# ethz-asl/ethzasl_brisk

Measured on AMD Instinct MI355X. Metric: frames/sec detect+describe @1080p (1/2/4/8 GPU); % HBM roofline, higher is better.
Workload: dtype u8

## Files before the change

ethzasl_brisk_amd/csrc/brisk_device_detect.h:

```cpp
#pragma once
#include "brisk_common.h"

BRISK_HD int brisk_min(int a, int b) { return a < b ? a : b; }
BRISK_HD int brisk_max(int a, int b) { return a > b ? a : b; }
BRISK_HD int brisk_min3(int a, int b, int c) { return brisk_min(brisk_min(a, b), c); }
BRISK_HD int brisk_max3(int a, int b, int c) { return brisk_max(brisk_max(a, b), c); }

struct BriskScoreBlock {
  uint32_t w0, w1, w2, w3;
  int x0, y0, cw, ch;
};

struct BriskLayerView {
  const uint8_t* img;
  uint16_t* smap;
  int w, h, stride;
  BriskScoreBlock blk;
  BriskScoreBlock blk58;
  mutable int miss;
};

BRISK_HD void brisk_block_clear(BriskScoreBlock* b) { b->w0 = b->w1 = b->w2 = b->w3 = 0; b->x0 = b->y0 = b->cw = b->ch = 0; }
BRISK_HD void brisk_block_from_bytes(BriskScoreBlock* b, const uint8_t* v, int n, int x0, int y0, int cw, int ch) {
  uint32_t w[4] = {0, 0, 0, 0};
  for (int i = 0; i < n; ++i) w[i >> 2] |= (uint32_t)v[i] << (8 * (i & 3));
  b->w0 = w[0]; b->w1 = w[1]; b->w2 = w[2]; b->w3 = w[3];
  b->x0 = x0; b->y0 = y0; b->cw = cw; b->ch = ch;
}
BRISK_HD int brisk_block_get(const BriskScoreBlock& b, int idx) {
  const uint32_t w = (idx < 8) ? ((idx < 4) ? b.w0 : b.w1) : ((idx < 12) ? b.w2 : b.w3);
  return (int)((w >> ((idx & 3) * 8)) & 0xFFu);
}

#if defined(__HIPCC__)
#ifdef BRISK_OUTLINE_HELPERS
#define BRISK_HD_OUTLINE __host__ __device__ static __attribute__((noinline))
#else
#define BRISK_HD_OUTLINE __host__ __device__ static inline
#endif
#else
#define BRISK_HD_OUTLINE static
#endif


BRISK_HD int brisk_avg(int a, int b) { return (a + b + 1) >> 1; }

BRISK_HD uint8_t brisk_half_px(const uint8_t* src, int sstride, int sw, int c, int r) {
  const uint8_t* p1 = src + (long)(2 * r) * sstride + 2 * c;
  const uint8_t* p2 = p1 + sstride;
  const int hsize = sw / 16;
  const int n1 = 16 * (hsize / 2);
  const int n2 = n1 + 8 * (hsize % 2);
  const int a = p1[0], b = p1[1], cc = p2[0], d = p2[1];
  if (c < n2) {
    const int v0 = brisk_avg(a, cc), v1 = brisk_avg(b, d);
    return (uint8_t)(c < n1 ? brisk_avg(v0, v1) : (v0 + v1) / 2);
  }
  return (uint8_t)((a + b + cc + d + 2) / 4);
}

BRISK_HD uint8_t brisk_twothird_px(const uint8_t* src, int sstride, int sw, int c, int r) {
  const int t = c >> 1, cx = c & 1;
  const int g = r >> 1, ry = r & 1;
  const uint8_t* pa = src + (long)(3 * g + (ry ? 2 : 0)) * sstride + 3 * t;
  const uint8_t* pb = src + (long)(3 * g + 1) * sstride + 3 * t;
  const int simd_cols = (sw / 15) * 10;
  const int o = cx ? 2 : 0;
  if (c < simd_cols) {
    const int uo = brisk_avg(brisk_avg(pa[o], pb[o]), pa[o]);
    const int um = brisk_avg(brisk_avg(pa[1], pb[1]), pa[1]);
    return (uint8_t)brisk_avg(brisk_avg(uo, um), uo);
  }
  const unsigned A1 = pa[o], A2 = pa[1], B1 = pb[o], B2 = pb[1];
  return (uint8_t)(((4 * A1 + 2 * (A2 + B1 + 1) + B2 + 1) / 9) & 0xFF);
}


BRISK_HD int brisk_oast9_16_M_from_d(const int* d) {
  int lo3[16], hi3[16];
#pragma unroll
  for (int i = 0; i < 16; ++i) {
    lo3[i] = brisk_min3(d[i], d[(i + 1) & 15], d[(i + 2) & 15]);
    hi3[i] = brisk_max3(d[i], d[(i + 1) & 15], d[(i + 2) & 15]);
  }
  int best_bright = -256, best_dark = 256;
#pragma unroll
  for (int i = 0; i < 16; ++i) {
    best_bright = brisk_max(best_bright, brisk_min3(lo3[i], lo3[(i + 3) & 15], lo3[(i + 6) & 15]));
    best_dark = brisk_min(best_dark, brisk_max3(hi3[i], hi3[(i + 3) & 15], hi3[(i + 6) & 15]));
  }
  return brisk_max(best_bright, -best_dark);
}

BRISK_HD int brisk_oast9_16_M(const uint8_t* p, int s) {
  const int c = p[0];
  int d[16];
  d[0] = p[-3] - c;          d[1] = p[-3 - s] - c;      d[2] = p[-2 - 2 * s] - c;  d[3] = p[-1 - 3 * s] - c;
  d[4] = p[-3 * s] - c;      d[5] = p[1 - 3 * s] - c;   d[6] = p[2 - 2 * s] - c;   d[7] = p[3 - s] - c;
  d[8] = p[3] - c;           d[9] = p[3 + s] - c;       d[10] = p[2 + 2 * s] - c;  d[11] = p[1 + 3 * s] - c;
  d[12] = p[3 * s] - c;      d[13] = p[-1 + 3 * s] - c; d[14] = p[-2 + 2 * s] - c; d[15] = p[-3 + s] - c;
  return brisk_oast9_16_M_from_d(d);
}

BRISK_HD int brisk_agast5_8_M_from_d(const int* d) {
  int best_bright = -256, best_dark = 256;
#pragma unroll
  for (int i = 0; i < 8; ++i) {
    const int lo = brisk_min(brisk_min3(d[i], d[(i + 1) & 7], d[(i + 2) & 7]), brisk_min(d[(i + 3) & 7], d[(i + 4) & 7]));
    const int hi = brisk_max(brisk_max3(d[i], d[(i + 1) & 7], d[(i + 2) & 7]), brisk_max(d[(i + 3) & 7], d[(i + 4) & 7]));
    best_bright = brisk_max(best_bright, lo);
    best_dark = brisk_min(best_dark, hi);
  }
  return brisk_max(best_bright, -best_dark);
}

BRISK_HD int brisk_agast5_8_M(const uint8_t* p, int s) {
  const int c = p[0];
  int d[8];
  d[0] = p[-1] - c; d[1] = p[-1 - s] - c; d[2] = p[-s] - c; d[3] = p[1 - s] - c;
  d[4] = p[1] - c;  d[5] = p[1 + s] - c;  d[6] = p[s] - c;  d[7] = p[-1 + s] - c;
  return brisk_agast5_8_M_from_d(d);
}

BRISK_HD int brisk_Kp_from_M(int M) { return brisk_min(brisk_max(M - 1, 0), 254); }

BRISK_HD void brisk_disc_minmax(const uint8_t* p, int s, int* mn_, int* mx_) {
  int mn = 255, mx = 0;
#pragma unroll
  for (int dy = -3; dy <= 3; ++dy) {
    const int r = (dy == -3 || dy == 3) ? 1 : (dy == -2 || dy == 2) ? 2 : 3;
    for (int dx = -r; dx <= r; ++dx) {
      const int v = p[dy * s + dx];
      mn = brisk_min(mn, v);
      mx = brisk_max(mx, v);
    }
  }
  *mn_ = mn;
  *mx_ = mx;
}

BRISK_HD float brisk_b2_factor(int thr) { return (float)thr * 0.01f; }
BRISK_HD int brisk_b2_fast(int tc, float k) {
#if defined(__HIP_DEVICE_COMPILE__)
  return (int)__fmaf_rn((float)tc, k, 0.005f);
#else
  return (int)fmaf((float)tc, k, 0.005f);
#endif
}

struct BriskPregate {
  uint32_t K;
  uint32_t shift;
  uint32_t lower;
};
BRISK_HD BriskPregate brisk_pregate_make(int thr, int lower_threshold = BRISK_LOWER_THRESHOLD) {
  int s = 8;
  while (s > 0 && 230 * ((thr << s) / 100) > 65535) --s;
  const uint32_t K = (uint32_t)((thr << s) / 100);
  BriskPregate g;
  g.K = K | (K << 16);
  g.shift = (uint32_t)s | ((uint32_t)s << 16);
  g.lower = (uint32_t)lower_threshold * 0x10001u;
  return g;
}

#if defined(__HIP_DEVICE_COMPILE__)
typedef short brisk_v2s __attribute__((ext_vector_type(2)));
typedef unsigned short brisk_v2u __attribute__((ext_vector_type(2)));
#define BRISK_PK_S(x) __builtin_bit_cast(brisk_v2s, (uint32_t)(x))
#define BRISK_PK_U(x) __builtin_bit_cast(brisk_v2u, (uint32_t)(x))
__device__ __forceinline__ uint32_t brisk_pk_sub(uint32_t a, uint32_t b) { return __builtin_bit_cast(uint32_t, (brisk_v2s)(BRISK_PK_S(a) - BRISK_PK_S(b))); }
__device__ __forceinline__ uint32_t brisk_pk_max(uint32_t a, uint32_t b) { return __builtin_bit_cast(uint32_t, __builtin_elementwise_max(BRISK_PK_S(a), BRISK_PK_S(b))); }
__device__ __forceinline__ uint32_t brisk_pk_min(uint32_t a, uint32_t b) { return __builtin_bit_cast(uint32_t, __builtin_elementwise_min(BRISK_PK_S(a), BRISK_PK_S(b))); }
__device__ __forceinline__ uint32_t brisk_pk_mul(uint32_t a, uint32_t b) { return __builtin_bit_cast(uint32_t, (brisk_v2u)(BRISK_PK_U(a) * BRISK_PK_U(b))); }
__device__ __forceinline__ uint32_t brisk_pk_shr(uint32_t a, uint32_t s) { return __builtin_bit_cast(uint32_t, (brisk_v2u)(BRISK_PK_U(a) >> BRISK_PK_U(s))); }
#else
#define BRISK_PK_LANES(expr)                                                              \
  const int a0 = (int16_t)(a & 0xFFFFu), a1 = (int16_t)(a >> 16);                         \
  const int b0 = (int16_t)(b & 0xFFFFu), b1 = (int16_t)(b >> 16);                         \
  (void)a0; (void)a1; (void)b0; (void)b1;                                                 \
  return expr;
static inline uint32_t brisk_pk_pack(int lo, int hi) { return ((uint32_t)lo & 0xFFFFu) | ((uint32_t)hi << 16); }
static inline uint32_t brisk_pk_sub(uint32_t a, uint32_t b) { BRISK_PK_LANES(brisk_pk_pack(a0 - b0, a1 - b1)) }
static inline uint32_t brisk_pk_max(uint32_t a, uint32_t b) { BRISK_PK_LANES(brisk_pk_pack(a0 > b0 ? a0 : b0, a1 > b1 ? a1 : b1)) }
static inline uint32_t brisk_pk_min(uint32_t a, uint32_t b) { BRISK_PK_LANES(brisk_pk_pack(a0 < b0 ? a0 : b0, a1 < b1 ? a1 : b1)) }
static inline uint32_t brisk_pk_mul(uint32_t a, uint32_t b) { return brisk_pk_pack((int)(((a & 0xFFFFu) * (b & 0xFFFFu)) & 0xFFFFu), (int)(((a >> 16) * (b >> 16)) & 0xFFFFu)); }
static inline uint32_t brisk_pk_shr(uint32_t a, uint32_t s) { return brisk_pk_pack((int)((a & 0xFFFFu) >> (s & 0xFFFFu)), (int)((a >> 16) >> (s >> 16))); }
#endif

#if defined(__HIP_DEVICE_COMPILE__)
__device__ __forceinline__ uint32_t brisk_pk_min_sw(uint32_t a, uint32_t b) {
  uint32_t r;
  asm("v_pk_min_i16 %0, %1, %2 op_sel:[0,1] op_sel_hi:[1,0]" : "=v"(r) : "v"(a), "v"(b));
  return r;
}
__device__ __forceinline__ uint32_t brisk_pk_max_sw(uint32_t a, uint32_t b) {
  uint32_t r;
  asm("v_pk_max_i16 %0, %1, %2 op_sel:[0,1] op_sel_hi:[1,0]" : "=v"(r) : "v"(a), "v"(b));
  return r;
}
#else
static inline uint32_t brisk_pk_min_sw(uint32_t a, uint32_t b) { return brisk_pk_min(a, (b >> 16) | (b << 16)); }
static inline uint32_t brisk_pk_max_sw(uint32_t a, uint32_t b) { return brisk_pk_max(a, (b >> 16) | (b << 16)); }
#endif

BRISK_HD uint32_t brisk_pk_ring_pair(uint32_t px_i, uint32_t px_i8, uint32_t centre_both) { return brisk_pk_sub(px_i | (px_i8 << 16), centre_both); }
BRISK_HD int brisk_oast9_16_M_from_pk(const uint32_t* P) {
  uint32_t lo2[8], hi2[8], lo4[8], hi4[8], lo8[8], hi8[8];
#pragma unroll
  for (int i = 0; i < 8; ++i) {
    lo2[i] = (i < 7) ? brisk_pk_min(P[i], P[i + 1]) : brisk_pk_min_sw(P[7], P[0]);
    hi2[i] = (i < 7) ? brisk_pk_max(P[i], P[i + 1]) : brisk_pk_max_sw(P[7], P[0]);
  }
#pragma unroll
  for (int i = 0; i < 8; ++i) {
    lo4[i] = (i < 6) ? brisk_pk_min(lo2[i], lo2[i + 2]) : brisk_pk_min_sw(lo2[i], lo2[i - 6]);
    hi4[i] = (i < 6) ? brisk_pk_max(hi2[i], hi2[i + 2]) : brisk_pk_max_sw(hi2[i], hi2[i - 6]);
  }
#pragma unroll
  for (int i = 0; i < 8; ++i) {
    lo8[i] = (i < 4) ? brisk_pk_min(lo4[i], lo4[i + 4]) : brisk_pk_min_sw(lo4[i], lo4[i - 4]);
    hi8[i] = (i < 4) ? brisk_pk_max(hi4[i], hi4[i + 4]) : brisk_pk_max_sw(hi4[i], hi4[i - 4]);
  }
  uint32_t bb = 0, bd = 0;
#pragma unroll
  for (int i = 0; i < 8; ++i) {
    const uint32_t lo9 = brisk_pk_min_sw(lo8[i], P[i]), hi9 = brisk_pk_max_sw(hi8[i], P[i]);
    bb = (i == 0) ? lo9 : brisk_pk_max(bb, lo9);
    bd = (i == 0) ? hi9 : brisk_pk_min(bd, hi9);
  }
  const int best_bright = brisk_max((int)(int16_t)(bb & 0xFFFFu), (int)(int16_t)(bb >> 16));
  const int best_dark = brisk_min((int)(int16_t)(bd & 0xFFFFu), (int)(int16_t)(bd >> 16));
  return brisk_max(best_bright, -best_dark);
}

BRISK_HD uint32_t brisk_pregate_pair(uint32_t c, uint32_t n, uint32_t s, uint32_t w, uint32_t e, const BriskPregate& g) {
  const uint32_t mxNS = brisk_pk_max(n, s), mnNS = brisk_pk_min(n, s);
  const uint32_t mxWE = brisk_pk_max(w, e), mnWE = brisk_pk_min(w, e);
  const uint32_t vb = brisk_pk_min(mxNS, mxWE);
  const uint32_t vd = brisk_pk_max(mnNS, mnWE);
  const uint32_t t5 = brisk_pk_sub(brisk_pk_max(mxNS, mxWE), brisk_pk_min(mnNS, mnWE));
  const uint32_t upper = (uint32_t)BRISK_UPPER_THRESHOLD * 0x10001u;
  const uint32_t tc = brisk_pk_min(brisk_pk_max(t5, g.lower), upper);
  const uint32_t b2p = brisk_pk_shr(brisk_pk_mul(tc, g.K), g.shift);
  const uint32_t ev = brisk_pk_max(brisk_pk_sub(vb, c), brisk_pk_sub(c, vd));
  return brisk_pk_sub(b2p, ev) & 0x80008000u;
}

BRISK_HD int brisk_detect_px(const uint8_t* p, int s, int thr, int lower = BRISK_LOWER_THRESHOLD) {
  int mn, mx;
  brisk_disc_minmax(p, s, &mn, &mx);
  const int t = mx - mn;
  const int cmp = (thr * lower) / 100;
  if (t < cmp) return 0;
  const int tc = brisk_min(brisk_max(t, lower), BRISK_UPPER_THRESHOLD);
  const int b2 = (tc * thr) / 100;
  const int c = p[0];
  if (mx - c <= b2 && c - mn <= b2) return 0;
  return brisk_oast9_16_M(p, s) > b2 ? t : 0;
}

BRISK_HD bool brisk_border3(const BriskLayerView& L, int x, int y) {
  return x < 3 || y < 3 || x >= L.w - 3 || y >= L.h - 3;
}

BRISK_HD int brisk_Kp(const BriskLayerView& L, int x, int y) {
  return brisk_Kp_from_M(brisk_oast9_16_M(L.img + (long)y * L.stride + x, L.stride));
}

BRISK_HD int brisk_V_eval(const BriskLayerView& L, int x, int y) {
  if (brisk_border3(L, x, y)) return 0;
  const int D = BRISK_SM_D(L.smap[(long)y * L.stride + x]);
  if (D > 2) return D;
  return brisk_Kp(L, x, y);
}
BRISK_HD int brisk_S_literal(const BriskLayerView& L, int x, int y, int threshold ) {
  if (x < 3 || y < 3) return 0;
  if (x >= L.w - 3 || y >= L.h - 3) return 0;
  uint16_t* sc = L.smap + (long)y * L.stride + x;
  const int m = (int)(*sc & 0xFFu);
  if (m > 2) return m;
  const int b = threshold - 1;
  const int M = brisk_oast9_16_M(L.img + (long)y * L.stride + x, L.stride);
  int score = (int)(uint8_t)brisk_max(b, brisk_min(M - 1, 254));
  if (score < threshold) score = 0;
  *sc = (uint16_t)score;
  return score;
}

template <int DIRECT>
BRISK_HD int brisk_V(const BriskLayerView& L, int x, int y) {
  if (DIRECT == 2) return brisk_S_literal(L, x, y, 1);
  if (DIRECT) return brisk_V_eval(L, x, y);
  const unsigned ux = (unsigned)(x - L.blk.x0), uy = (unsigned)(y - L.blk.y0);
  if (ux < (unsigned)L.blk.cw && uy < (unsigned)L.blk.ch) return brisk_block_get(L.blk, (int)(uy * L.blk.cw + ux));
  L.miss = 1;
  return 0;
}

BRISK_HD int brisk_V58_eval(const BriskLayerView& L, int x, int y) {
  if (x < 2 || y < 2 || x >= L.w - 2 || y >= L.h - 2) return 0;
  return brisk_Kp_from_M(brisk_agast5_8_M(L.img + (long)y * L.stride + x, L.stride));
}
template <int DIRECT>
BRISK_HD int brisk_V58(const BriskLayerView& L, int x, int y) {
  if (DIRECT) return brisk_V58_eval(L, x, y);
  const unsigned ux = (unsigned)(x - L.blk58.x0), uy = (unsigned)(y - L.blk58.y0);
  if (L.blk58.cw && ux < 3u && uy < 3u) return brisk_block_get(L.blk58, (int)(uy * 3 + ux));
  L.miss = 1;
  return 0;
}

BRISK_HD void brisk_block_anchor(bool above, bool odd, int x_layer, int y_layer, int* ax, int* ay) {
  if (above) {
    if (!odd) {
      *ax = (4 * x_layer - 3) / 6 - 1;
      *ay = (4 * y_layer - 3) / 6 - 1;
    } else {
      *ax = (6 * x_layer - 4) / 8 - 1;
      *ay = (6 * y_layer - 4) / 8 - 1;
    }
  } else {
    if (!odd) {
      *ax = (8 * x_layer - 3) / 6;
      *ay = (8 * y_layer - 3) / 6;
    } else {
      *ax = (6 * x_layer - 2) / 4;
      *ay = (6 * y_layer - 2) / 4;
    }
  }
}

struct BriskTouch {
  int x0, y0;
  unsigned mask;
  bool on;
#ifdef CR_TIMING
  long long tlast;
  int tacc[6];
#endif
};
#if defined(CR_TIMING) && defined(__HIP_DEVICE_COMPILE__)
#define BRISK_CR_T(t_, i_) { const long long now_ = (long long)wall_clock64(); (t_)->tacc[i_] += (int)(now_ - (t_)->tlast); (t_)->tlast = now_; }
#else
#define BRISK_CR_T(t_, i_)
#endif

BRISK_HD void brisk_touch(BriskTouch* t, const BriskLayerView& L, int x, int y) {
  if (!t->on || brisk_border3(L, x, y)) return;
  const int bx = x - t->x0, by = y - t->y0;
  if (bx >= 0 && bx < 4 && by >= 0 && by < 4) t->mask |= 1u << (by * 4 + bx);
}

template <int DIRECT>
BRISK_HD int brisk_Vt(const BriskLayerView& L, int x, int y, BriskTouch* t) {
  brisk_touch(t, L, x, y);
  return brisk_V<DIRECT>(L, x, y);
}

BRISK_HD int brisk_bilinear_u8(const float rx1, const float ry1, const int s00, const int s10, const int s01, const int s11) {
  const float rx = 1.0f - rx1;
  const float ry = 1.0f - ry1;
  return (int)(uint8_t)(rx * ry * s00 + rx1 * ry * s10 + rx * ry1 * s01 + rx1 * ry1 * s11);
}
template <int DIRECT>
BRISK_HD int brisk_Vf(const BriskLayerView& L, float xf, float yf, BriskTouch* t) {
  const int x = (int)xf;
  const float rx1 = xf - (float)x;
  const int y = (int)yf;
  const float ry1 = yf - (float)y;
  const int s00 = brisk_Vt<DIRECT>(L, x, y, t);
  const int s10 = brisk_Vt<DIRECT>(L, x + 1, y, t);
  const int s01 = brisk_Vt<DIRECT>(L, x, y + 1, t);
  const int s11 = brisk_Vt<DIRECT>(L, x + 1, y + 1, t);
  return brisk_bilinear_u8(rx1, ry1, s00, s10, s01, s11);
}

struct BriskQuadric {
  int A, B, C, D, E, F;
};
BRISK_HD float brisk_quadric_at(const BriskQuadric& q, float x, float y) {
  return (q.A * x * x + q.B * y * y + q.C * x + q.D * y + q.E * x * y + q.F) / 18.0f;
}
BRISK_HD float brisk_clamp_unit(float v) { return v > 1.0f ? 1.0f : (v < -1.0f ? -1.0f : v); }

BRISK_HD_OUTLINE float brisk_subpixel2d(const int s_0_0, const int s_0_1, const int s_0_2, const int s_1_0,
                                const int s_1_1, const int s_1_2, const int s_2_0, const int s_2_1,
                                const int s_2_2, float& delta_x, float& delta_y) {
  const int left = s_0_0 + s_0_1 + s_0_2, right = s_2_0 + s_2_1 + s_2_2, mid_col = s_1_0 + s_1_1 + s_1_2;
  const int top = s_0_0 + s_1_0 + s_2_0, bottom = s_0_2 + s_1_2 + s_2_2, mid_row = s_0_1 + s_1_1 + s_2_1;
  BriskQuadric q;
  q.A = 3 * (left + right - 2 * mid_col);
  q.B = 3 * (top + bottom - 2 * mid_row);
  q.C = 3 * (right - left);
  q.D = 3 * (bottom - top);
  q.E = 4 * (s_0_0 - s_0_2 - s_2_0 + s_2_2);
  q.F = 2 * (5 * s_1_1 + 2 * (s_1_0 + s_0_1 + s_1_2 + s_2_1) - (s_0_0 + s_0_2 + s_2_0 + s_2_2));
  const int det = 4 * q.A * q.B - q.E * q.E;
  if (det == 0) {
    delta_x = 0.0f;
// ... 1170 lines not shown
```

ethzasl_brisk_amd/csrc/brisk_kernels.hip:

```cpp
#include <hip/hip_runtime.h>
#include <stdlib.h>

#include "brisk_common.h"
#include "brisk_device_detect.h"
#include "brisk_kernels.h"

#ifdef BRISK_HIP_TUNING
static int env_knob(const char* name, int dflt) {
  const char* v = getenv(name);
  return (v && *v) ? atoi(v) : dflt;
}
#else
#define env_knob(name, dflt) (dflt)
#endif


__device__ __forceinline__ BriskLayerView make_view(const BriskGeom& G, uint8_t* pyr, uint16_t* smap, int frame,
                                                    int l) {
  BriskLayerView v;
  const long base = (long)frame * G.pyr_elems + G.L[l].off;
  v.img = brisk_layer_img(G, pyr, frame, l);
  v.smap = smap + base;
  v.w = G.L[l].w;
  v.h = G.L[l].h;
// ... 238 lines not shown
      if (gy < h) {
        if (!full)
          for (int q = 0; q < 4; ++q)
            if (gx + q < w) v |= (unsigned)src[(long)gy * row_pitch + gx + q] << (8 * q);
        if (gx < s0 && !G.l0_ext) *reinterpret_cast<unsigned*>(L0 + (long)gy * s0 + gx) = v;
      }
      *reinterpret_cast<unsigned*>(&t0[i * 4]) = v;
    }
  }
  __syncthreads();
  if (threadIdx.x < 192) {
    const int cq = threadIdx.x % 24, rg = threadIdx.x / 24;
    unsigned lo = 0, hi = 0;
#pragma unroll
    for (int r = 0; r < 12; ++r) {
      const unsigned v = *reinterpret_cast<const unsigned*>(&t0[(rg * 12 + r) * 96 + cq * 4]);
      lo += v & 0x00FF00FFu;
      hi += (v >> 8) & 0x00FF00FFu;
    }
    psum[rg][cq] = make_uint2(lo, hi);
  }
  {
    const TileRef st = {t0, bx, by, 96};
    if (even_levels >= 1)
      pyramid_tile_level<false>(tile_origin(st), 96, w, P + G.L[2].off, G.L[2].stride, G.L[2].w, G.L[2].h, bx >> 1, by >> 1, 48, t2);
    if (odd_levels >= 0)
      pyramid_tile_level<true>(tile_origin(st), 96, w, P + G.L[1].off, G.L[1].stride, G.L[1].w, G.L[1].h, bx / 3 * 2, by / 3 * 2, 64, t1);
  }
  __syncthreads();
  if (threadIdx.x < 96) {
    const int c = threadIdx.x, cq = c >> 2, k = c & 3;
    unsigned tot = 0;
#pragma unroll
    for (int rg = 0; rg < 8; ++rg) {
      const uint2 p = psum[rg][cq];
      const unsigned w = (k & 1) ? p.y : p.x;
      tot += (k & 2) ? (w >> 16) : (w & 0xFFFFu);
    }
    uint32_t* row = bandsum + ((long)frame * tiles_y + by / PF_BAND) * istride;
    if (bx + c + 1 < istride) row[bx + c + 1] = tot;
    if (bx == 0 && c == 0) row[0] = 0;
  }
  {
    const TileRef s2 = {t2, bx >> 1, by >> 1, 48}, s1 = {t1, bx / 3 * 2, by / 3 * 2, 64};
    if (even_levels >= 2)
      pyramid_tile_level<false>(tile_origin(s2), 48, G.L[2].w, P + G.L[4].off, G.L[4].stride, G.L[4].w, G.L[4].h, bx >> 2, by >> 2, 24, t4);
    if (odd_levels >= 1)
      pyramid_tile_level<false>(tile_origin(s1), 64, G.L[1].w, P + G.L[3].off, G.L[3].stride, G.L[3].w, G.L[3].h, bx / 3, by / 3, 32, t3);
  }
  __syncthreads();
  {
    const TileRef s4 = {t4, bx >> 2, by >> 2, 24}, s3 = {t3, bx / 3, by / 3, 32};
    if (even_levels >= 3)
      pyramid_tile_level<false>(tile_origin(s4), 24, G.L[4].w, P + G.L[6].off, G.L[6].stride, G.L[6].w, G.L[6].h, bx >> 3, by >> 3, 12, nullptr);
    if (odd_levels >= 2)
      pyramid_tile_level<false>(tile_origin(s3), 32, G.L[3].w, P + G.L[5].off, G.L[5].stride, G.L[5].w, G.L[5].h, bx / 6, by / 6, 16, t5);
  }
  __syncthreads();
  if (odd_levels >= 3) {
    const TileRef s5 = {t5, bx / 6, by / 6, 16};
    pyramid_tile_level<false>(tile_origin(s5), 16, G.L[5].w, P + G.L[7].off, G.L[7].stride, G.L[7].w, G.L[7].h, bx / 12, by / 12, 8, nullptr);
  }
}

#define DT_W BRISK_DETECT_TILE_W
#define DT_H BRISK_DETECT_TILE_H
#define DT_R BRISK_DETECT_ROWS_PER_THREAD
#define DT_PITCH 80
#define DT_ROWDW ((DT_W + 8) / 4)
#define DT_LH (DT_H + 6)
#define DT_WR (DT_R + 6)
#define DT_NLD ((DT_LH * DT_ROWDW + 255) / 256)
static_assert(DT_H == 16 * DT_R && DT_W == 64, "256 threads = 16 column groups x 16 row groups");

__device__ __forceinline__ int wave_inclusive_scan(int v) {
  v += __builtin_amdgcn_update_dpp(0, v, 0x111, 0xf, 0xf, false);
  v += __builtin_amdgcn_update_dpp(0, v, 0x112, 0xf, 0xf, false);
  v += __builtin_amdgcn_update_dpp(0, v, 0x114, 0xf, 0xf, false);
  v += __builtin_amdgcn_update_dpp(0, v, 0x118, 0xf, 0xf, false);
  v += __builtin_amdgcn_update_dpp(0, v, 0x142, 0xa, 0xf, false);
  v += __builtin_amdgcn_update_dpp(0, v, 0x143, 0xc, 0xf, false);
  return v;
}

__global__ void __launch_bounds__(256) k_detect(BriskGeom G, BriskTileTable T, const uint8_t* __restrict__ pyr,
                                                 uint16_t* __restrict__ smap, BriskCand* __restrict__ cand,
                                                 BriskFrameCounters* __restrict__ counters, int cand_cap) {
  __shared__ __attribute__((aligned(16))) uint8_t tile[DT_LH * DT_PITCH];
  __shared__ uint16_t queue[DT_H * DT_W];
  __shared__ int qcount;
  const int frame = blockIdx.y;
#ifdef DT_TIMING
  unsigned long long dt_last = __builtin_amdgcn_s_memtime();
  unsigned dt_acc[7] = {0, 0, 0, 0, 0, 0, 0};
  asm volatile("s_waitcnt lgkmcnt(0)" ::: "memory");
#define DT_T(i) do { const unsigned long long t_ = __builtin_amdgcn_s_memtime(); asm volatile("s_waitcnt lgkmcnt(0)" ::: "memory"); dt_acc[i] += (unsigned)(t_ - dt_last); dt_last = t_; } while (0)
#else
#define DT_T(i) do { } while (0)
#endif
  const int nt = T.total_tiles;
  const int res = ((blockIdx.x & 7) + frame) & 7;
  const int slot = blockIdx.x >> 3;
  if (slot >= (nt >> 3) + (res < (nt & 7) ? 1 : 0)) return;
  const int tid_sw = res * (nt >> 3) + min(res, nt & 7) + slot;
  int l = 0;
  while (l + 1 < G.nlayers && tid_sw >= T.first_tile[l + 1]) ++l;
  const int t = tid_sw - T.first_tile[l];
  const int tx = t % T.tiles_x[l], ty = t / T.tiles_x[l];
  const int w = G.L[l].w, h = G.L[l].h, stride = G.L[l].stride;
  const long base = (long)frame * G.pyr_elems + G.L[l].off;
  const uint8_t* img = brisk_layer_img(G, pyr, frame, l);
  const int x0 = tx * DT_W, y0 = ty * DT_H;
  const int thr = G.threshold;

  {
    constexpr int DT_RG = 256 / DT_ROWDW;
    static_assert(DT_RG * DT_NLD >= DT_LH, "the row groups cover the halo tile");
    unsigned stg[DT_NLD];
    const int col = threadIdx.x % DT_ROWDW, rg = threadIdx.x / DT_ROWDW;
    const uint8_t* colp = img + min(max(x0 - 4 + col * 4, 0), stride - 4);
#pragma unroll
    for (int k = 0; k < DT_NLD; ++k) {
      const int rr = min(rg + DT_RG * k, DT_LH - 1);
      const int cy = min(max(y0 - 3 + rr, 0), h - 1);
      stg[k] = *reinterpret_cast<const unsigned*>(colp + (long)cy * stride);
    }
    uint8_t* tp = &tile[rg * DT_PITCH + col * 4];
#pragma unroll
    for (int k = 0; k < DT_NLD; ++k)
      if (rg < DT_RG && rg + DT_RG * k < DT_LH) *reinterpret_cast<unsigned*>(tp + DT_RG * k * DT_PITCH) = stg[k];
  }
  if (threadIdx.x == 0) qcount = 0;
  DT_T(0);
  __syncthreads();
  DT_T(1);

  const int lx = (threadIdx.x & 15) * 4, ly = (threadIdx.x >> 4) * DT_R;
  const int lane = threadIdx.x & 63;
  {
    const BriskPregate pg = brisk_pregate_make(thr, G.lower_threshold);
    unsigned R[DT_WR][3];
#pragma unroll
    for (int r = 0; r < DT_WR; ++r) {
      const unsigned* p = reinterpret_cast<const unsigned*>(&tile[(ly + r) * DT_PITCH + lx]);
      R[r][0] = p[0]; R[r][1] = p[1]; R[r][2] = p[2];
    }
    unsigned CA[DT_WR], CB[DT_WR];
#pragma unroll
    for (int r = 0; r < DT_WR; ++r) {
      CA[r] = __builtin_amdgcn_perm(0u, R[r][1], 0x0c010c00u);
      CB[r] = __builtin_amdgcn_perm(0u, R[r][1], 0x0c030c02u);
    }
    DT_T(2);
    unsigned m = 0;
#pragma unroll
    for (int rr = 0; rr < DT_R; ++rr) {
      const int ci = rr + 3;
      const unsigned WA = __builtin_amdgcn_perm(0u, R[ci][0], 0x0c020c01u);
      const unsigned WB = __builtin_amdgcn_perm(R[ci][1], R[ci][0], 0x0c040c03u);
      const unsigned EA = __builtin_amdgcn_perm(R[ci][2], R[ci][1], 0x0c040c03u);
      const unsigned EB = __builtin_amdgcn_perm(0u, R[ci][2], 0x0c020c01u);
      const unsigned gA = brisk_pregate_pair(CA[ci], CA[rr], CA[rr + 6], WA, EA, pg);
      const unsigned gB = brisk_pregate_pair(CB[ci], CB[rr], CB[rr + 6], WB, EB, pg);
      m = (m >> 1) | gA;
      m = (m >> 1) | gB;
    }
    DT_T(3);
    const int cnt = __popc(m);
    const int incl = wave_inclusive_scan(cnt);
    const int total = __builtin_amdgcn_readlane(incl, 63);
    if (total) {
      int qb = 0;
      if (lane == 0) qb = atomicAdd(&qcount, total);
      qb = __builtin_amdgcn_readfirstlane(qb);
      int pos = qb + incl - cnt;
      while (m) {
        const int bit = __ffs(m) - 1;
        m &= m - 1;
        const int k = (bit & 15) - (16 - 2 * DT_R), half = bit >> 4;
        queue[pos++] = (uint16_t)((ly + (k >> 1)) * DT_W + lx + ((k & 1) << 1) + half);
      }
    }
  }
  DT_T(4);
  __syncthreads();
  DT_T(5);

  const int nq = qcount;
  const int cmp = (thr * G.lower_threshold) / 100;
  const float kthr = brisk_b2_factor(thr);
  for (int i = threadIdx.x; i < nq; i += 256) {
    const int idx = queue[i];
    const int py = idx / DT_W, px = idx % DT_W;
    const int gx = x0 + px, gyy = y0 + py;
    if (gx < 3 || gyy < 3 || gx > w - 4 || gyy > h - 4) continue;
    const uint8_t* p = &tile[(py + 3) * DT_PITCH + px + 4];
    int v[7][7];
#pragma unroll
    for (int dy = -3; dy <= 3; ++dy) {
      const int hw = (dy == -3 || dy == 3) ? 1 : (dy == -2 || dy == 2) ? 2 : 3;
#pragma unroll
      for (int dx = -3; dx <= 3; ++dx) v[dy + 3][dx + 3] = (dx >= -hw && dx <= hw) ? (int)p[dy * DT_PITCH + dx] : -1;
    }
    int mx = 0, mn = 255;
#pragma unroll
    for (int dy = 0; dy < 7; ++dy)
#pragma unroll
      for (int dx = 0; dx < 7; ++dx)
        if (v[dy][dx] >= 0) { mx = max(mx, v[dy][dx]); mn = min(mn, v[dy][dx]); }
    const int tt = mx - mn;
    if (tt < cmp) continue;
    const int tc = min(max(tt, G.lower_threshold), BRISK_UPPER_THRESHOLD);
    const int b2 = brisk_b2_fast(tc, kthr);
    const int c = v[3][3];
    if (mx - c <= b2 && c - mn <= b2) continue;
    const uint32_t cc = (uint32_t)c * 0x10001u;
    uint32_t P[8];
    P[0] = brisk_pk_ring_pair(v[3][0], v[3][6], cc); P[1] = brisk_pk_ring_pair(v[2][0], v[4][6], cc);
    P[2] = brisk_pk_ring_pair(v[1][1], v[5][5], cc); P[3] = brisk_pk_ring_pair(v[0][2], v[6][4], cc);
    P[4] = brisk_pk_ring_pair(v[0][3], v[6][3], cc); P[5] = brisk_pk_ring_pair(v[0][4], v[6][2], cc);
    P[6] = brisk_pk_ring_pair(v[1][5], v[5][1], cc); P[7] = brisk_pk_ring_pair(v[2][6], v[4][0], cc);
    if (brisk_oast9_16_M_from_pk(P) > b2) {
      const int D = tt;
      smap[base + (long)gyy * stride + gx] = (uint16_t)D;
      if (D <= 2) counters[frame].low_score = 1;
      const int ci = atomicAdd(&counters[frame].ncand, 1);
      if (ci < cand_cap) {
        BriskCand cnd;
        cnd.x = (uint16_t)gx; cnd.y = (uint16_t)gyy; cnd.layer = (uint8_t)l; cnd.D = (uint8_t)D;
        cnd.status = 0; cnd.flags = 0; cnd.fp_x0 = 0; cnd.fp_y0 = 0; cnd.fp_mask = 0; cnd.pad = 0;
        cnd.kx = cnd.ky = cnd.ksize = cnd.kresp = 0.f;
        cnd.key = ((unsigned)l << 26) | ((unsigned)gyy << 13) | (unsigned)gx;
        cand[(long)frame * cand_cap + ci] = cnd;
      } else {
        atomicOr(&counters[frame].overflow, 1);
      }
    }
  }
  DT_T(6);
#ifdef DT_TIMING
  if ((threadIdx.x & 63) == 0 && ((blockIdx.x >> 3) & 15) == 3) {
    for (int k = 0; k < 7; ++k) atomicAdd(&counters[frame].tdet[k], (int)dt_acc[k]);
    atomicAdd(&counters[frame].tdet[7], 1);
  }
#endif
}

__global__ void __launch_bounds__(256) k_smap_clear(BriskGeom G, uint16_t* __restrict__ smap, const BriskCand* __restrict__ cand,
                                                    const BriskFrameCounters* __restrict__ counters, int cand_cap) {
  const int frame = blockIdx.y;
  uint16_t* fs = smap + (long)frame * G.pyr_elems;
  const int ncand = counters[frame].ncand;
  if (ncand > cand_cap || (counters[frame].overflow & 1) || counters[frame].full_clear) {
    uint4* p = reinterpret_cast<uint4*>(fs);
    const long n16 = (long)G.pyr_elems * 2 / 16;
    for (long i = (long)blockIdx.x * blockDim.x + threadIdx.x; i < n16; i += (long)gridDim.x * blockDim.x) p[i] = make_uint4(0, 0, 0, 0);
    return;
  }
  for (int i = blockIdx.x * blockDim.x + threadIdx.x; i < ncand; i += gridDim.x * blockDim.x) {
    const BriskCand c = cand[(long)frame * cand_cap + i];
    const int l = c.layer;
    fs[G.L[l].off + (long)c.y * G.L[l].stride + c.x] = 0;
    if (c.fp_mask && l + 1 < G.nlayers) {
      uint16_t* a = fs + G.L[l + 1].off;
      const int st = G.L[l + 1].stride;
      for (int b = 0; b < 16; ++b)
        if (c.fp_mask & (1u << b)) a[(long)(c.fp_y0 + (b >> 2)) * st + c.fp_x0 + (b & 3)] = 0;
    }
  }
}

#define SB_WAVES 4
#ifndef SB_PER_WAVE
#define SB_PER_WAVE 3
#endif
__device__ __forceinline__ constexpr int sb_dx16(int j) { constexpr int t[16] = {-3, -3, -2, -1, 0, 1, 2, 3, 3, 3, 2, 1, 0, -1, -2, -3}; return t[j]; }
__device__ __forceinline__ constexpr int sb_dy16(int j) { constexpr int t[16] = {0, -1, -2, -3, -3, -3, -2, -1, 0, 1, 2, 3, 3, 3, 2, 1}; return t[j]; }
__device__ __forceinline__ constexpr int sb_dx8(int j) { constexpr int t[8] = {-1, -1, 0, 1, 1, 1, 0, -1}; return t[j]; }
__device__ __forceinline__ constexpr int sb_dy8(int j) { constexpr int t[8] = {0, -1, -1, -1, 0, 1, 1, 1}; return t[j]; }

#define SB_PROWS 11
#define SB_PSLOTS (3 * SB_PROWS * 4)

__global__ void __launch_bounds__(SB_WAVES * 64) k_score_blocks(BriskGeom G, const uint8_t* __restrict__ pyr,
                                                                const uint16_t* __restrict__ smap,
                                                                const BriskCand* __restrict__ cand,
                                                                const BriskFrameCounters* __restrict__ counters,
                                                                uint8_t* __restrict__ blocks, int cand_cap, int nframes, int bpf) {
  int frame, bx;
  if (!xcd_frame_block(nframes, bpf, &frame, &bx)) return;
  const int wave = threadIdx.x >> 6, lane = threadIdx.x & 63;
  if (counters[frame].low_score) return;
  const int n = min(counters[frame].ncand, cand_cap);
  const uint8_t* fimg = pyr + (long)frame * G.pyr_elems;
  const uint8_t* img0 = G.l0_ext ? G.l0_ext + (long)frame * G.l0_pitch : nullptr;
  const uint16_t* fsm = smap + (long)frame * G.pyr_elems;
  const int role = (lane < 25) ? 0 : (lane >= 32 && lane < 48) ? 1 : (lane >= 48) ? 2 : 3;
  __shared__ int4 lgeo[BRISK_MAX_LAYERS];
  __shared__ __attribute__((aligned(16))) uint8_t patch[SB_WAVES][SB_PER_WAVE][3][SB_PROWS][16];
  if (threadIdx.x < BRISK_MAX_LAYERS) lgeo[threadIdx.x] = make_int4(G.L[threadIdx.x].w, G.L[threadIdx.x].h, G.L[threadIdx.x].stride, G.L[threadIdx.x].off);
  __syncthreads();
#ifdef SB_TIMING
  int sb_acc[4] = {0, 0, 0, 0};
  long long sb_last = (long long)wall_clock64();
#define SB_T(i) { const long long now_ = (long long)wall_clock64(); sb_acc[i] += (int)(now_ - sb_last); sb_last = now_; }
#else
#define SB_T(i)
#endif
  for (int base = (bx * SB_WAVES + wave) * SB_PER_WAVE; base < n; base += bpf * SB_WAVES * SB_PER_WAVE) {
    uint2 hdr[SB_PER_WAVE];
#pragma unroll
    for (int k = 0; k < SB_PER_WAVE; ++k)
      hdr[k] = *reinterpret_cast<const uint2*>(&cand[(long)frame * cand_cap + min(base + k, n - 1)]);
    unsigned pv[SB_PER_WAVE][3];
    unsigned smv[SB_PER_WAVE];
    int cofs[SB_PER_WAVE];
    bool ok[SB_PER_WAVE], is8[SB_PER_WAVE];
#pragma unroll
    for (int k = 0; k < SB_PER_WAVE; ++k) {
      const int hx = __builtin_amdgcn_readfirstlane((int)hdr[k].x);
      const int x = hx & 0xFFFF, y = (int)((unsigned)hx >> 16);
      const int l = __builtin_amdgcn_readfirstlane((int)(hdr[k].y & 0xFF));
      const bool has_above = !G.single_layer && (l + 1 < G.nlayers);
      const bool has_below = !G.single_layer && (l > 0);
      const bool has_58 = !G.single_layer && (l == 0);
      int ax = 0, ay = 0, bx = 0, by = 0;
      brisk_block_anchor(true, (l & 1) != 0, x, y, &ax, &ay);
      brisk_block_anchor(false, (l & 1) != 0, x, y, &bx, &by);
      const int ox0 = x - 5, oy0 = y - 5, ox1 = ax - 3, oy1 = ay - 3, ox2 = bx - 3, oy2 = by - 3;
#pragma unroll
      for (int t = 0; t < 3; ++t) {
        const int r = min(lane >> 2, SB_PROWS - 1), d = lane & 3;
        const int pl = (t == 0) ? l : (t == 1) ? (has_above ? l + 1 : l) : (has_below ? l - 1 : l);
        const int pw = G.L[pl].stride, ph = G.L[pl].h;
        const int pox = (t == 0) ? ox0 : (t == 1) ? ox1 : ox2;
        const int poy = (t == 0) ? oy0 : (t == 1) ? oy1 : oy2;
        const int gx = min(max((pox & ~3) + 4 * d, 0), pw - 4);
        const int gy = min(max(poy + r, 0), ph - 1);
        const uint8_t* limg = (pl == 0 && img0) ? img0 : fimg + G.L[pl].off;
        pv[k][t] = *reinterpret_cast<const unsigned*>(limg + (gy * pw + gx));
      }
      int ll = l, px = 0, py = 0, which = 0;
      bool valid = false;
      is8[k] = false;
      if (role == 0) {
        px = x - 2 + lane % 5; py = y - 2 + lane / 5; valid = true;
      } else if (role == 1) {
        ll = has_above ? l + 1 : l; px = ax + (lane & 3); py = ay + ((lane - 32) >> 2); valid = has_above; which = 1;
      } else if (role == 2) {
        const int p = lane - 48;
        if (has_below) {
          ll = l - 1; px = bx + (p & 3); py = by + (p >> 2); valid = true; which = 2;
        } else if (has_58 && p < 9) {
          px = x - 1 + p % 3; py = y - 1 + p / 3; valid = true; is8[k] = true;
        }
      }
      const int4 gg = lgeo[ll];
      const int w = gg.x, h = gg.y, st = gg.z, off = gg.w;
      const int bd = is8[k] ? 2 : 3;
      ok[k] = valid && px >= bd && py >= bd && px < w - bd && py < h - bd;
      smv[k] = fsm[(long)off + (ok[k] ? (long)py * st + px : 0)];
      const int pox = (which == 0) ? ox0 : (which == 1) ? ox1 : ox2;
      const int poy = (which == 0) ? oy0 : (which == 1) ? oy1 : oy2;
      cofs[k] = which * (SB_PROWS * 16) + (py - poy) * 16 + (px - (pox & ~3));
    }
    SB_T(0)
#pragma unroll
    for (int k = 0; k < SB_PER_WAVE; ++k)
#pragma unroll
      for (int t = 0; t < 3; ++t)
        if (lane < SB_PROWS * 4) *reinterpret_cast<unsigned*>(&patch[wave][k][t][0][0] + lane * 4) = pv[k][t];
    __builtin_amdgcn_fence(__ATOMIC_RELEASE, "wavefront");
    __builtin_amdgcn_wave_barrier();
    __builtin_amdgcn_fence(__ATOMIC_ACQUIRE, "wavefront");
    SB_T(1)
#pragma unroll
    for (int k = 0; k < SB_PER_WAVE; ++k) {
      const uint8_t* pc = &patch[wave][k][0][0][0] + (ok[k] ? cofs[k] : 5 * 16 + 8);
      const int c = pc[0];
      uint32_t P[8];
      const uint32_t cc = (uint32_t)c * 0x10001u;
#pragma unroll
      for (int i = 0; i < 8; ++i) {
        const uint32_t a = pc[sb_dx16(i) + sb_dy16(i) * 16], b = pc[sb_dx16(i + 8) + sb_dy16(i + 8) * 16];
        P[i] = brisk_pk_ring_pair(a, b, cc);
      }
      int v = brisk_Kp_from_M(brisk_oast9_16_M_from_pk(P));
      const int D = BRISK_SM_D(smv[k]);
      if (D > 2) v = D;
      if (__any(is8[k])) {
        int d8[8];
#pragma unroll
        for (int j = 0; j < 8; ++j) d8[j] = (int)pc[sb_dx8(j) + sb_dy8(j) * 16] - c;
        const int v8 = brisk_Kp_from_M(brisk_agast5_8_M_from_d(d8));
        if (is8[k]) v = v8;
      }
      if (!ok[k]) v = 0;
      if (base + k < n) blocks[((long)frame * cand_cap + base + k) * 64 + lane] = (uint8_t)v;
    }
    __builtin_amdgcn_wave_barrier();
    SB_T(2)
#ifdef SB_TIMING
    sb_acc[3] += 1;
#endif
  }
#ifdef SB_TIMING
  if (lane == 0) for (int i = 0; i < 4; ++i) atomicAdd(const_cast<int*>(&counters[frame].sphase[i]), sb_acc[i]);
#endif
}

__global__ void __launch_bounds__(64) k_classify_refine(BriskGeom G, uint8_t* pyr, uint16_t* smap, BriskCand* cand,
                                                         BriskFrameCounters* counters, const uint8_t* blocks, int* tie_idx,
                                                         int cand_cap, int tie_cap, int nframes, int bpf) {
  int frame, bx;
  if (!xcd_frame_block(nframes, bpf, &frame, &bx)) return;
  if (counters[frame].low_score) return;
  const int n = min(counters[frame].ncand, cand_cap);
  for (int mine = bx * blockDim.x + threadIdx.x; mine < n; mine += bpf * blockDim.x) {
#ifdef CR_TIMING
    const long long cr_t0 = (long long)wall_clock64();
#endif
    BriskCand* c = &cand[(long)frame * cand_cap + mine];
    const int x = c->x, y = c->y, l = c->layer, D = c->D;
    const bool has_above = !G.single_layer && (l + 1 < G.nlayers);
    const bool has_below = !G.single_layer && (l > 0);
    const bool has_58 = !G.single_layer && (l == 0);
    BriskLayerView Lo = make_view(G, pyr, smap, frame, l);
    BriskLayerView La = make_view(G, pyr, smap, frame, has_above ? l + 1 : l);
    BriskLayerView Lb = make_view(G, pyr, smap, frame, has_below ? l - 1 : l);
    const uint4* blk = reinterpret_cast<const uint4*>(blocks + ((long)frame * cand_cap + mine) * 64);
    const uint4 o = blk[0], o2 = blk[1], a = blk[2], b = blk[3];
    {
      const unsigned w1 = o.y, w2 = o.z, w3 = o.w, w4 = o2.x;
      Lo.blk.w0 = ((w1 >> 16) & 0xFFFFu) | ((w2 & 0xFFu) << 16) | (w2 & 0xFF000000u);
      Lo.blk.w1 = (w3 & 0xFFFFu) | ((w4 & 0xFFFFu) << 16);
      Lo.blk.w2 = (w4 >> 16) & 0xFFu;
      Lo.blk.w3 = 0;
      Lo.blk.x0 = x - 1; Lo.blk.y0 = y - 1; Lo.blk.cw = 3; Lo.blk.ch = 3;
    }
    if (has_58) { Lo.blk58.w0 = b.x; Lo.blk58.w1 = b.y; Lo.blk58.w2 = b.z; Lo.blk58.w3 = b.w; Lo.blk58.x0 = x - 1; Lo.blk58.y0 = y - 1; Lo.blk58.cw = 3; Lo.blk58.ch = 3; }
    if (has_above) {
      int ax, ay;
      brisk_block_anchor(true, (l & 1) != 0, x, y, &ax, &ay);
      La.blk.w0 = a.x; La.blk.w1 = a.y; La.blk.w2 = a.z; La.blk.w3 = a.w; La.blk.x0 = ax; La.blk.y0 = ay; La.blk.cw = 4; La.blk.ch = 4;
    }
    if (has_below) {
      int bx, by;
      brisk_block_anchor(false, (l & 1) != 0, x, y, &bx, &by);
      Lb.blk.w0 = b.x; Lb.blk.w1 = b.y; Lb.blk.w2 = b.z; Lb.blk.w3 = b.w; Lb.blk.x0 = bx; Lb.blk.y0 = by; Lb.blk.cw = 4; Lb.blk.ch = 4;
    }
    int nprobed = 0;
    unsigned flags = 0;
    BriskKeyPoint kp;
    kp.x = kp.y = kp.size = kp.response = 0.f;
    BriskTouch touch;
    touch.on = false; touch.mask = 0; touch.x0 = 0; touch.y0 = 0;
#ifdef CR_TIMING
    touch.tlast = cr_t0;
    for (int i = 0; i < 6; ++i) touch.tacc[i] = 0;
#endif
    bool e5 = false;
    const unsigned status = brisk_classify<false>(Lo, x, y, D, &nprobed);
    BRISK_CR_T(&touch, 0)
    if (status != BRISK_ST_REJ && brisk_refine<false>(G, Lb, Lo, La, l, x, y, &kp, &e5, &touch)) flags |= 1;
#ifdef CR_TIMING
    { const long long now_ = (long long)wall_clock64(); atomicAdd(&counters[frame].cphase[7], (int)(now_ - touch.tlast)); touch.tlast = now_; }
#endif
    if ((Lo.miss | La.miss | Lb.miss) || (BRISK_DBG_FLAGS(G) & 1)) {
      c->status = 0xFF;
      atomicAdd(&counters[frame].nredo, 1);
      continue;
    }
    int tie_j = 0;
    if (status == BRISK_ST_TIE) tie_j = atomicAdd(&counters[frame].ntie[l], 1);
    unsigned bits = ((unsigned)nprobed << 8) | (status << 12);
    if (e5) { flags |= 2; bits |= BRISK_SM_E5; }
    if (flags & 1) { c->kx = kp.x; c->ky = kp.y; c->ksize = kp.size; c->kresp = kp.response; }
    c->fp_x0 = (int16_t)touch.x0; c->fp_y0 = (int16_t)touch.y0; c->fp_mask = (uint16_t)touch.mask;
    c->status = (uint8_t)status;
    c->flags = (uint8_t)flags;
    if (status == BRISK_ST_PASS && touch.mask) {
      for (int bb = 0; bb < 16; ++bb)
        if (touch.mask & (1u << bb)) smap_or(La.smap, (long)(touch.y0 + (bb >> 2)) * La.stride + touch.x0 + (bb & 3), BRISK_SM_TOUCH);
    }
    smap_or(Lo.smap, (long)y * Lo.stride + x, bits);
    if (status == BRISK_ST_TIE) {
      if (tie_j < tie_cap) tie_idx[((long)frame * BRISK_MAX_LAYERS + l) * tie_cap + tie_j] = mine;
      else atomicOr(&counters[frame].overflow, 2);
    }
#ifdef CR_TIMING
    BRISK_CR_T(&touch, 5)
    for (int i = 0; i < 6; ++i) atomicAdd(&counters[frame].cphase[i], touch.tacc[i]);
    atomicAdd(&counters[frame].cphase[6], 1);
#endif
  }
}

__global__ void __launch_bounds__(64) k_classify_refine_direct(BriskGeom G, uint8_t* pyr, uint16_t* smap, BriskCand* cand,
                                                                BriskFrameCounters* counters, int* tie_idx, int cand_cap,
                                                                int tie_cap) {
  const int frame = blockIdx.y;
  if (counters[frame].nredo == 0 || counters[frame].low_score) return;
  const int n = min(counters[frame].ncand, cand_cap);
  for (int i = blockIdx.x * blockDim.x + threadIdx.x; i < n; i += gridDim.x * blockDim.x) {
    BriskCand* c = &cand[(long)frame * cand_cap + i];
    if (c->status != 0xFF) continue;
    const int l = c->layer, x = c->x, y = c->y, D = c->D;
    const bool has_above = !G.single_layer && (l + 1 < G.nlayers);
    const bool has_below = !G.single_layer && (l > 0);
    const BriskLayerView Lo = make_view(G, pyr, smap, frame, l);
    const BriskLayerView La = make_view(G, pyr, smap, frame, has_above ? l + 1 : l);
    const BriskLayerView Lb = make_view(G, pyr, smap, frame, has_below ? l - 1 : l);
    int nprobed = 0;
    unsigned flags = 0;
    BriskKeyPoint kp;
    kp.x = kp.y = kp.size = kp.response = 0.f;
    BriskTouch touch;
    touch.on = false; touch.mask = 0; touch.x0 = 0; touch.y0 = 0;
    bool e5 = false;
    const unsigned status = brisk_classify<true>(Lo, x, y, D, &nprobed);
    if (status != BRISK_ST_REJ && brisk_refine<true>(G, Lb, Lo, La, l, x, y, &kp, &e5, &touch)) flags |= 1;
    unsigned bits = ((unsigned)nprobed << 8) | (status << 12);
    if (e5) { flags |= 2; bits |= BRISK_SM_E5; }
    if (flags & 1) { c->kx = kp.x; c->ky = kp.y; c->ksize = kp.size; c->kresp = kp.response; }
    c->fp_x0 = (int16_t)touch.x0; c->fp_y0 = (int16_t)touch.y0; c->fp_mask = (uint16_t)touch.mask;
    c->status = (uint8_t)status;
    c->flags = (uint8_t)flags;
    if (status == BRISK_ST_PASS && touch.mask) {
      for (int b = 0; b < 16; ++b)
        if (touch.mask & (1u << b)) smap_or(La.smap, (long)(touch.y0 + (b >> 2)) * La.stride + touch.x0 + (b & 3), BRISK_SM_TOUCH);
    }
    if (status == BRISK_ST_TIE) {
      const int j = atomicAdd(&counters[frame].ntie[l], 1);
      if (j < tie_cap) tie_idx[((long)frame * BRISK_MAX_LAYERS + l) * tie_cap + j] = i;
      else atomicOr(&counters[frame].overflow, 2);
    }
    smap_or(Lo.smap, (long)y * Lo.stride + x, bits);
  }
}

// ... 915 lines not shown
```

Baseline: 78660.

## Compute OAST arc extrema with prefix/suffix scans and defer centre subtraction

Replaces the three-level doubling min/max network for 9-of-16 arc extrema with prefix and suffix min/max scans over the eight packed ring pairs. It works on raw pixel values and subtracts the centre only once at the end, which removes eight packed subtracts per candidate. The pregate pass-flag packing now uses a byte permute into a column-by-row bitmask with a simpler decode, in place of the interleaved shift-or. The new scans have to reproduce the old arc semantics exactly; any mistake there would silently change which keypoints are detected.

```diff
diff --git a/ethzasl_brisk_amd/csrc/brisk_device_detect.h b/ethzasl_brisk_amd/csrc/brisk_device_detect.h
--- a/ethzasl_brisk_amd/csrc/brisk_device_detect.h
+++ b/ethzasl_brisk_amd/csrc/brisk_device_detect.h
@@ -174,6 +174,7 @@
 __device__ __forceinline__ uint32_t brisk_pk_min(uint32_t a, uint32_t b) { return __builtin_bit_cast(uint32_t, __builtin_elementwise_min(BRISK_PK_S(a), BRISK_PK_S(b))); }
 __device__ __forceinline__ uint32_t brisk_pk_mul(uint32_t a, uint32_t b) { return __builtin_bit_cast(uint32_t, (brisk_v2u)(BRISK_PK_U(a) * BRISK_PK_U(b))); }
 __device__ __forceinline__ uint32_t brisk_pk_shr(uint32_t a, uint32_t s) { return __builtin_bit_cast(uint32_t, (brisk_v2u)(BRISK_PK_U(a) >> BRISK_PK_U(s))); }
+__device__ __forceinline__ uint32_t brisk_high_bytes(uint32_t lo, uint32_t hi) { return __builtin_amdgcn_perm(hi, lo, 0x07050301u); }
 #else
 #define BRISK_PK_LANES(expr)                                                              \
   const int a0 = (int16_t)(a & 0xFFFFu), a1 = (int16_t)(a >> 16);                         \
@@ -186,6 +187,9 @@
 static inline uint32_t brisk_pk_min(uint32_t a, uint32_t b) { BRISK_PK_LANES(brisk_pk_pack(a0 < b0 ? a0 : b0, a1 < b1 ? a1 : b1)) }
 static inline uint32_t brisk_pk_mul(uint32_t a, uint32_t b) { return brisk_pk_pack((int)(((a & 0xFFFFu) * (b & 0xFFFFu)) & 0xFFFFu), (int)(((a >> 16) * (b >> 16)) & 0xFFFFu)); }
 static inline uint32_t brisk_pk_shr(uint32_t a, uint32_t s) { return brisk_pk_pack((int)((a & 0xFFFFu) >> (s & 0xFFFFu)), (int)((a >> 16) >> (s >> 16))); }
+static inline uint32_t brisk_high_bytes(uint32_t lo, uint32_t hi) {
+  return ((lo >> 8) & 0xFFu) | ((lo >> 16) & 0xFF00u) | ((hi << 8) & 0xFF0000u) | (hi & 0xFF000000u);
+}
 #endif
 
 #if defined(__HIP_DEVICE_COMPILE__)
@@ -204,37 +208,49 @@
 static inline uint32_t brisk_pk_max_sw(uint32_t a, uint32_t b) { return brisk_pk_max(a, (b >> 16) | (b << 16)); }
 #endif
 
-BRISK_HD uint32_t brisk_pk_ring_pair(uint32_t px_i, uint32_t px_i8, uint32_t centre_both) { return brisk_pk_sub(px_i | (px_i8 << 16), centre_both); }
-BRISK_HD int brisk_oast9_16_M_from_pk(const uint32_t* P) {
-  uint32_t lo2[8], hi2[8], lo4[8], hi4[8], lo8[8], hi8[8];
+BRISK_HD void brisk_oast9_16_arcs_pk(const uint32_t* P, uint32_t* bb_, uint32_t* bd_) {
+  uint32_t Smin[8], Smax[8], Pmin[8], Pmax[8];
+  Smin[7] = Smax[7] = P[7];
+#pragma unroll
+  for (int i = 6; i >= 0; --i) {
+    Smin[i] = brisk_pk_min(P[i], Smin[i + 1]);
+    Smax[i] = brisk_pk_max(P[i], Smax[i + 1]);
+  }
+  Pmin[0] = Pmax[0] = P[0];
+#pragma unroll
+  for (int i = 1; i < 7; ++i) {
+    Pmin[i] = brisk_pk_min(P[i], Pmin[i - 1]);
+    Pmax[i] = brisk_pk_max(P[i], Pmax[i - 1]);
+  }
+  Pmin[7] = Smin[0];
+  Pmax[7] = Smax[0];
+  uint32_t bb = 0, bd = 0;
 #pragma unroll
   for (int i = 0; i < 8; ++i) {
-    lo2[i] = (i < 7) ? brisk_pk_min(P[i], P[i + 1]) : brisk_pk_min_sw(P[7], P[0]);
-    hi2[i] = (i < 7) ? brisk_pk_max(P[i], P[i + 1]) : brisk_pk_max_sw(P[7], P[0]);
-  }
-#pragma unroll
-  for (int i = 0; i < 8; ++i) {
-    lo4[i] = (i < 6) ? brisk_pk_min(lo2[i], lo2[i + 2]) : brisk_pk_min_sw(lo2[i], lo2[i - 6]);
-    hi4[i] = (i < 6) ? brisk_pk_max(hi2[i], hi2[i + 2]) : brisk_pk_max_sw(hi2[i], hi2[i - 6]);
-  }
-#pragma unroll
-  for (int i = 0; i < 8; ++i) {
-    lo8[i] = (i < 4) ? brisk_pk_min(lo4[i], lo4[i + 4]) : brisk_pk_min_sw(lo4[i], lo4[i - 4]);
-    hi8[i] = (i < 4) ? brisk_pk_max(hi4[i], hi4[i + 4]) : brisk_pk_max_sw(hi4[i], hi4[i - 4]);
-  }
-  uint32_t bb = 0, bd = 0;
-#pragma unroll
-  for (int i = 0; i < 8; ++i) {
-    const uint32_t lo9 = brisk_pk_min_sw(lo8[i], P[i]), hi9 = brisk_pk_max_sw(hi8[i], P[i]);
+    const uint32_t lo9 = brisk_pk_min_sw(Smin[i], Pmin[i]), hi9 = brisk_pk_max_sw(Smax[i], Pmax[i]);
     bb = (i == 0) ? lo9 : brisk_pk_max(bb, lo9);
     bd = (i == 0) ? hi9 : brisk_pk_min(bd, hi9);
   }
+  *bb_ = bb;
+  *bd_ = bd;
+}
+BRISK_HD int brisk_oast9_16_M_from_pk(const uint32_t* P) {
+  uint32_t bb, bd;
+  brisk_oast9_16_arcs_pk(P, &bb, &bd);
   const int best_bright = brisk_max((int)(int16_t)(bb & 0xFFFFu), (int)(int16_t)(bb >> 16));
   const int best_dark = brisk_min((int)(int16_t)(bd & 0xFFFFu), (int)(int16_t)(bd >> 16));
   return brisk_max(best_bright, -best_dark);
 }
-
-BRISK_HD uint32_t brisk_pregate_pair(uint32_t c, uint32_t n, uint32_t s, uint32_t w, uint32_t e, const BriskPregate& g) {
+BRISK_HD uint32_t brisk_pk_ring_pair(uint32_t px_i, uint32_t px_i8) { return px_i | (px_i8 << 16); }
+BRISK_HD int brisk_oast9_16_M_from_px(const uint32_t* Q, int c) {
+  uint32_t bb, bd;
+  brisk_oast9_16_arcs_pk(Q, &bb, &bd);
+  const int best_bright = brisk_max((int)(bb & 0xFFFFu), (int)(bb >> 16)) - c;
+  const int best_dark = brisk_min((int)(bd & 0xFFFFu), (int)(bd >> 16)) - c;
+  return brisk_max(best_bright, -best_dark);
+}
+
+BRISK_HD uint32_t brisk_pregate_pair_d(uint32_t c, uint32_t n, uint32_t s, uint32_t w, uint32_t e, const BriskPregate& g) {
   const uint32_t mxNS = brisk_pk_max(n, s), mnNS = brisk_pk_min(n, s);
   const uint32_t mxWE = brisk_pk_max(w, e), mnWE = brisk_pk_min(w, e);
   const uint32_t vb = brisk_pk_min(mxNS, mxWE);
@@ -244,8 +260,20 @@
   const uint32_t tc = brisk_pk_min(brisk_pk_max(t5, g.lower), upper);
   const uint32_t b2p = brisk_pk_shr(brisk_pk_mul(tc, g.K), g.shift);
   const uint32_t ev = brisk_pk_max(brisk_pk_sub(vb, c), brisk_pk_sub(c, vd));
-  return brisk_pk_sub(b2p, ev) & 0x80008000u;
-}
+  return brisk_pk_sub(b2p, ev);
+}
+BRISK_HD uint32_t brisk_pregate_pair(uint32_t c, uint32_t n, uint32_t s, uint32_t w, uint32_t e, const BriskPregate& g) {
+  return brisk_pregate_pair_d(c, n, s, w, e, g) & 0x80008000u;
+}
+
+BRISK_HD uint32_t brisk_pregate_flags_row(uint32_t acc, uint32_t d01, uint32_t d23, int rr) {
+  const uint32_t f = brisk_high_bytes(d01, d23);
+  if (rr == 0) return f;
+  const uint32_t sel = 0x80808080u >> rr;
+  return (acc & ~sel) | ((f >> rr) & sel);
+}
+BRISK_HD uint32_t brisk_pregate_flags_mask(uint32_t acc, int rows) { return acc & (0x01010101u * ((0xFF00u >> rows) & 0xFFu)); }
+BRISK_HD void brisk_pregate_flags_decode(int bit, int* col, int* row) { *col = bit >> 3; *row = 7 - (bit & 7); }
 
 BRISK_HD int brisk_detect_px(const uint8_t* p, int s, int thr, int lower = BRISK_LOWER_THRESHOLD) {
   int mn, mx;
diff --git a/ethzasl_brisk_amd/csrc/brisk_kernels.hip b/ethzasl_brisk_amd/csrc/brisk_kernels.hip
--- a/ethzasl_brisk_amd/csrc/brisk_kernels.hip
+++ b/ethzasl_brisk_amd/csrc/brisk_kernels.hip
@@ -414,6 +414,7 @@
       CB[r] = __builtin_amdgcn_perm(0u, R[r][1], 0x0c030c02u);
     }
     DT_T(2);
+    static_assert(DT_R <= 8, "a byte of the pass flags holds one column's rows");
     unsigned m = 0;
 #pragma unroll
     for (int rr = 0; rr < DT_R; ++rr) {
@@ -422,11 +423,11 @@
       const unsigned WB = __builtin_amdgcn_perm(R[ci][1], R[ci][0], 0x0c040c03u);
       const unsigned EA = __builtin_amdgcn_perm(R[ci][2], R[ci][1], 0x0c040c03u);
       const unsigned EB = __builtin_amdgcn_perm(0u, R[ci][2], 0x0c020c01u);
-      const unsigned gA = brisk_pregate_pair(CA[ci], CA[rr], CA[rr + 6], WA, EA, pg);
-      const unsigned gB = brisk_pregate_pair(CB[ci], CB[rr], CB[rr + 6], WB, EB, pg);
-      m = (m >> 1) | gA;
-      m = (m >> 1) | gB;
-    }
+      const unsigned gA = brisk_pregate_pair_d(CA[ci], CA[rr], CA[rr + 6], WA, EA, pg);
+      const unsigned gB = brisk_pregate_pair_d(CB[ci], CB[rr], CB[rr + 6], WB, EB, pg);
+      m = brisk_pregate_flags_row(m, gA, gB, rr);
+    }
+    m = brisk_pregate_flags_mask(m, DT_R);
     DT_T(3);
     const int cnt = __popc(m);
     const int incl = wave_inclusive_scan(cnt);
@@ -439,8 +440,9 @@
       while (m) {
         const int bit = __ffs(m) - 1;
         m &= m - 1;
-        const int k = (bit & 15) - (16 - 2 * DT_R), half = bit >> 4;
-        queue[pos++] = (uint16_t)((ly + (k >> 1)) * DT_W + lx + ((k & 1) << 1) + half);
+        int col, row;
+        brisk_pregate_flags_decode(bit, &col, &row);
+        queue[pos++] = (uint16_t)((ly + row) * DT_W + lx + col);
       }
     }
   }
@@ -476,13 +478,12 @@
     const int b2 = brisk_b2_fast(tc, kthr);
     const int c = v[3][3];
     if (mx - c <= b2 && c - mn <= b2) continue;
-    const uint32_t cc = (uint32_t)c * 0x10001u;
     uint32_t P[8];
-    P[0] = brisk_pk_ring_pair(v[3][0], v[3][6], cc); P[1] = brisk_pk_ring_pair(v[2][0], v[4][6], cc);
-    P[2] = brisk_pk_ring_pair(v[1][1], v[5][5], cc); P[3] = brisk_pk_ring_pair(v[0][2], v[6][4], cc);
-    P[4] = brisk_pk_ring_pair(v[0][3], v[6][3], cc); P[5] = brisk_pk_ring_pair(v[0][4], v[6][2], cc);
-    P[6] = brisk_pk_ring_pair(v[1][5], v[5][1], cc); P[7] = brisk_pk_ring_pair(v[2][6], v[4][0], cc);
-    if (brisk_oast9_16_M_from_pk(P) > b2) {
+    P[0] = brisk_pk_ring_pair(v[3][0], v[3][6]); P[1] = brisk_pk_ring_pair(v[2][0], v[4][6]);
+    P[2] = brisk_pk_ring_pair(v[1][1], v[5][5]); P[3] = brisk_pk_ring_pair(v[0][2], v[6][4]);
+    P[4] = brisk_pk_ring_pair(v[0][3], v[6][3]); P[5] = brisk_pk_ring_pair(v[0][4], v[6][2]);
+    P[6] = brisk_pk_ring_pair(v[1][5], v[5][1]); P[7] = brisk_pk_ring_pair(v[2][6], v[4][0]);
+    if (brisk_oast9_16_M_from_px(P, c) > b2) {
       const int D = tt;
       smap[base + (long)gyy * stride + gx] = (uint16_t)D;
       if (D <= 2) counters[frame].low_score = 1;
@@ -641,13 +642,12 @@
       const uint8_t* pc = &patch[wave][k][0][0][0] + (ok[k] ? cofs[k] : 5 * 16 + 8);
       const int c = pc[0];
       uint32_t P[8];
-      const uint32_t cc = (uint32_t)c * 0x10001u;
 #pragma unroll
       for (int i = 0; i < 8; ++i) {
         const uint32_t a = pc[sb_dx16(i) + sb_dy16(i) * 16], b = pc[sb_dx16(i + 8) + sb_dy16(i + 8) * 16];
-        P[i] = brisk_pk_ring_pair(a, b, cc);
+        P[i] = brisk_pk_ring_pair(a, b);
       }
-      int v = brisk_Kp_from_M(brisk_oast9_16_M_from_pk(P));
+      int v = brisk_Kp_from_M(brisk_oast9_16_M_from_px(P, c));
       const int D = BRISK_SM_D(smv[k]);
       if (D > 2) v = D;
       if (__any(is8[k])) {
```

Result: faster. 80200, median of 6 (+2.0%).
